# pmelchior/scarlet

Hardware: AMD Instinct MI355X
Metric: PGM iters/sec over batched blends; achieved HBM GB/s vs roofline (higher is better)
Workload: dtype f32; 1 GPU; configs[2]: 1024 independent 5-band 128x128 blends in total, 10 ExtendedSource components (41x41) each, ConvolutionRenderer FFT 160x160; iterations 0..1234 of a fit from the initial parameters; loop=blend, blends_total=1024, components_per_blend=10, sub_ranges_per_gpu=3

## Files before the change

scarlet_amd/csrc/fused_conv.hip:

```cpp
#include <cstdlib>
#include <type_traits>

#include "common.h"
#include "fft_regs.h"

namespace smi {

using fftk::cf;
using fftk::cmul;
using fftk::cmulc;
using fftk::ld;
using fftk::st;

namespace {

#ifndef SMI_CONV_THREADS
#define SMI_CONV_THREADS 1024
#endif
constexpr int kThreads = SMI_CONV_THREADS;
constexpr int kF2 = 16;

constexpr int conv_column_stride(int fy) { return ((fy + fy / kF2 + 3) / 8) * 8 + 4; }
constexpr size_t conv_lds_bytes(int fy, int fx) {
    return sizeof(float2) * ((size_t)(fx / 2) * conv_column_stride(fy) + 2 * fy + fx) +
           sizeof(double) * (kThreads / 64);
}

template <int FY1, int FX1, int ZB>
struct Cfg {
    static constexpr int FY = FY1 * kF2, FX = FX1 * kF2;
    static constexpr int NY1 = FY1 - ZB, NX1 = FX1 - ZB;
    static_assert(ZB >= 0 && NY1 >= 1 && NX1 >= 1, "padding blocks");
    static constexpr int NKX = FX / 2 + 1, NT = FX / 2;
    static constexpr int SY = conv_column_stride(FY);
    static_assert(SY >= FY + FY / kF2 && SY % 8 == 4, "column stride");
    static constexpr size_t lds_bytes = conv_lds_bytes(FY, FX);
};

__device__ __forceinline__ int sk(int y) { return y + (y >> 4); }

template <int F1, bool INV, int LIVE>
__device__ __forceinline__ void pass_stride_col(float2 *a, int n2, const cf (&tw)[F1]) {
    cf v[F1];
#pragma unroll
    for (int n1 = 0; n1 < F1; ++n1) {
        v[n1] = (INV || n1 < LIVE) ? ld(a[(kF2 + 1) * n1 + n2]) : cf{0.f, 0.f};
        if (INV && n1 > 0) v[n1] = cmulc(v[n1], tw[n1]);
    }
    fftk::Dft<F1, INV>::run(v);
#pragma unroll
    for (int k1 = 0; k1 < F1; ++k1) {
        if (INV && k1 >= LIVE) continue;
        if (!INV && k1 > 0) v[k1] = cmul(v[k1], tw[k1]);
        a[(kF2 + 1) * k1 + n2] = st(v[k1]);
    }
}

__device__ __forceinline__ void wave_lds_fence() {
    asm volatile("s_waitcnt lgkmcnt(0)" ::: "memory");
}

__host__ __device__ __forceinline__ int column_of(int kx, int Fx) {
    const int fx1 = Fx / kF2;
    return 2 * kx == Fx ? kx : 8 * (kx % fx1) + kx / fx1;
}

template <int F1>
__device__ __forceinline__ int pos(int k) {
    return kF2 * (k % F1) + k / F1;
}

__device__ __forceinline__ void wave_partial(double v, double *part) {
    for (int o = 32; o > 0; o >>= 1) v += __shfl_xor(v, o, 64);
    if ((threadIdx.x & 63) == 0) part[threadIdx.x >> 6] = v;
}
__device__ __forceinline__ double sum_partials(const double *part) {
    double t = 0.0;
    for (int i = 0; i < kThreads / 64; ++i) t += part[i];
    return t;
}

__device__ __forceinline__ void lds_barrier() {
    asm volatile("s_waitcnt lgkmcnt(0)\n\ts_barrier" ::: "memory");
}

using plane_t = __amdgpu_buffer_rsrc_t;
__device__ __forceinline__ plane_t band_plane(const float *p, int n_elements) {
    return __builtin_amdgcn_make_buffer_rsrc(const_cast<float *>(p), 0, n_elements * 4, 0x00020000);
}
__device__ __forceinline__ void plane_store(plane_t r, int y, int x, int W, float value) {
    const uint32_t off = x < W ? (uint32_t)(y * W + x) * 4u : 0x80000000u;
    __builtin_amdgcn_raw_buffer_store_b32(__builtin_bit_cast(uint32_t, value), r, off, 0, 0);
}
__device__ __forceinline__ float plane_load(plane_t r, int y, int x, int W) {
    const uint32_t off = x < W ? (uint32_t)(y * W + x) * 4u : 0x80000000u;
    return __builtin_bit_cast(float, __builtin_amdgcn_raw_buffer_load_b32(r, off, 0, 0));
}
struct PairRows {
    uint32_t o0, o1;
};
__device__ __forceinline__ PairRows pair_rows(int y, int n2, int W) {
    PairRows a;
    a.o0 = (uint32_t)(y * W + n2) * 4u;
    a.o1 = a.o0 + (uint32_t)W * 4u;
    asm volatile("" : "+v"(a.o0), "+v"(a.o1));
    return a;
}
template <int N1>
__device__ __forceinline__ void dw_load(const char *plane, uint32_t o, cf &d, cf &w) {
    const float4 t = *reinterpret_cast<const float4 *>(plane + (size_t)o + 16u * kF2 * N1);
    d = cf{t.x, t.y};
    w = cf{t.z, t.w};
}
template <int N1>
__device__ __forceinline__ cf pair_load(plane_t r, PairRows a) {
    return cf{__builtin_bit_cast(float, __builtin_amdgcn_raw_buffer_load_b32(r, a.o0 + 4u * kF2 * N1, 0, 0)),
              __builtin_bit_cast(float, __builtin_amdgcn_raw_buffer_load_b32(r, a.o1 + 4u * kF2 * N1, 0, 0))};
}

template <int FY1, int FX1, int ZB>
struct Conv {
    using C = Cfg<FY1, FX1, ZB>;
    static constexpr int NX1 = C::NX1;
    float2 *T, *twy, *twx, *qtab;
    int tid, n_pairs;

    __device__ __forceinline__ void zero_tail(float2 *a, int g) const {
        for (int y = 2 * n_pairs + g; y < kF2 * C::NY1; y += kF2) a[sk(y)] = make_float2(0.f, 0.f);
    }

    __device__ __forceinline__ void columns(const float2 *Kt, bool conj) {
        const int g = tid & (kF2 - 1), G = tid >> 4;
        const int col = 8 * (G >> 3) + ((G >> 1) & 3) + 4 * (G & 1);
        constexpr int kStep = kThreads / kF2;
        cf tw[FY1];
#pragma unroll
        for (int k1 = 0; k1 < FY1; ++k1) tw[k1] = ld(twy[kF2 * k1 + g]);
        for (int kt = col; kt < C::NT; kt += kStep) {
            const int kx = kt < 32 ? kt ^ 16 : kt;
            float2 *a = T + kx * C::SY;
            pass_stride_col<FY1, false, C::NY1>(a, g, tw);
            wave_lds_fence();
            if (g < FY1) {
                float2 *blk = a + (kF2 + 1) * g;
                const float2 *kp = Kt + (int64_t)kx * C::FY + kF2 * g;
                cf v[kF2], kv[kF2];
#pragma unroll
                for (int j = 0; j < kF2; ++j) kv[j] = ld(kp[j]);
#pragma unroll
                for (int j = 0; j < kF2; ++j) v[j] = ld(blk[j]);
                fftk::Dft<kF2, false>::run(v);
                if (kx == 0) {
#pragma unroll
                    for (int j = 0; j < kF2; ++j) blk[j] = st(v[j]);
                }
#pragma unroll
                for (int j = 0; j < kF2; ++j) v[j] = conj ? cmulc(v[j], kv[j]) : cmul(v[j], kv[j]);
                if (kx == 0) {
                    wave_lds_fence();
                    const float2 *base = g == 0 ? a + 1 : a + (kF2 + 1) * (FY1 - g);
                    const float2 *base0 = g == 0 ? a - 15 : base;
                    const float2 *qb = qtab + kF2 * g;
#pragma unroll
                    for (int j = 0; j < kF2; ++j) {
                        const cf m = ld((j == 0 ? base0 : base)[15 - j]), q = ld(qb[j]);
                        v[j] += conj ? cmul(cf{q.x, -q.y}, cf{m.x, -m.y}) : cmulc(q, m);
                        if (j % 4 == 3) __builtin_amdgcn_sched_barrier(0);
                    }
                    wave_lds_fence();
                }
                fftk::Dft<kF2, true>::run(v);
#pragma unroll
                for (int j = 0; j < kF2; ++j) blk[j] = st(v[j]);
            }
            wave_lds_fence();
            pass_stride_col<FY1, true, C::NY1>(a, g, tw);
            zero_tail(a, g);
        }
        lds_barrier();
    }

    struct StrideItem {
        int j, n2, zb;
        bool on;
    };
    __device__ __forceinline__ StrideItem stride_item(int it) const {
        StrideItem s;
        s.n2 = it & 15;
        s.j = it >> 4;
        s.on = s.j < n_pairs;
        s.zb = (s.n2 >> 1) * C::SY + sk(2 * s.j + (s.n2 & 1));
        return s;
    }
    __device__ __forceinline__ int stride_items() const { return n_pairs * kF2; }
    __device__ __forceinline__ void stride_twiddles(cf (&tw)[FX1], const StrideItem &s) const {
#pragma unroll
        for (int k1 = 1; k1 < FX1; ++k1) tw[k1] = ld(twx[kF2 * k1 + s.n2]);
    }
    __device__ __forceinline__ void stride_forward(cf *v, const StrideItem &s, const cf (&tw)[FX1]) {
        float2 *a = T + s.zb;
#pragma unroll
        for (int n1 = NX1; n1 < FX1; ++n1) v[n1] = cf{0.f, 0.f};
        fftk::Dft<FX1, false>::run(v);
#pragma unroll
        for (int k1 = 0; k1 < FX1; ++k1) {
            if (k1 > 0) v[k1] = cmul(v[k1], tw[k1]);
            a[8 * C::SY * k1] = st(v[k1]);
        }
    }
    __device__ __forceinline__ void stride_forward(cf *v, const StrideItem &s) {
        cf tw[FX1];
        stride_twiddles(tw, s);
        stride_forward(v, s, tw);
    }
    __device__ __forceinline__ void stride_inverse(cf *v, const StrideItem &s, const cf (&tw)[FX1]) {
        const float2 *a = T + s.zb;
#pragma unroll
        for (int n1 = 0; n1 < FX1; ++n1) {
            v[n1] = ld(a[8 * C::SY * n1]);
            if (n1 > 0) v[n1] = cmulc(v[n1], tw[n1]);
        }
        fftk::Dft<FX1, true>::run(v);
    }
    __device__ __forceinline__ void stride_inverse(cf *v, const StrideItem &s) {
        cf tw[FX1];
        stride_twiddles(tw, s);
        stride_inverse(v, s, tw);
    }

    static constexpr int kDouble = (FX1 - 1) / 2;
    static constexpr int kSlots = FX1 + (FX1 & 1);
    static constexpr int kGroupsPerTrip = (kThreads / 32) / kSlots;
    static_assert(kGroupsPerTrip >= 1, "slots of a pair group in one trip");
    static __device__ __forceinline__ int slot_block(int slot) {
        if (slot < 2 * kDouble) return (slot & 1) ? FX1 - (slot / 2 + 1) : slot / 2 + 1;
        return slot == 2 * kDouble ? 0 : FX1 / 2;
    }
    struct BlockItem {
        int z;
        int kind;
        bool wave_on;
    };
    BlockItem first;
    __device__ __forceinline__ BlockItem block_item(int group0) const {
        BlockItem b;
        const int grp = tid >> 5;
        const int slot = grp % kSlots;
        int j = (tid & 31) + 32 * (group0 + grp / kSlots);
        const int wgrp = __builtin_amdgcn_readfirstlane(tid >> 6) * 2;
        b.wave_on = wgrp < kGroupsPerTrip * kSlots && 32 * (group0 + wgrp / kSlots) < n_pairs;
        if (j >= n_pairs) j = n_pairs - 1;
        const int k1 = slot < FX1 ? slot_block(slot) : 0;
        b.z = 8 * k1 * C::SY + sk(2 * j);
        b.kind = slot < 2 * kDouble ? 0 : k1 == 0 ? 1 : 2;
        return b;
    }
    __device__ __forceinline__ void first_block_item() {
        first = block_item(0);
        asm volatile("" : "+v"(first.z), "+v"(first.kind));
    }
    __device__ __forceinline__ BlockItem trip_item(int trip) const {
        return trip == 0 ? first : block_item(trip * kGroupsPerTrip);
    }
    __device__ __forceinline__ int block_trips() const {
        if (kGroupsPerTrip >= (C::FY / 2 + 31) / 32) return 1;
        return ((n_pairs + 31) / 32 + kGroupsPerTrip - 1) / kGroupsPerTrip;
    }
    static __device__ __forceinline__ cf from_partner(cf v) {
        return cf{__shfl_xor(v.x, 32, 64), __shfl_xor(v.y, 32, 64)};
    }
    static __device__ __forceinline__ void sep(cf za, cf zb, cf &xa, cf &xb) {
        asm("v_pk_add_f32 %0, %1, %2 neg_hi:[0,1]" : "=v"(xa) : "v"(za), "v"(zb));
        asm("v_pk_add_f32 %0, %1, %2 op_sel:[1,1] op_sel_hi:[0,0] neg_hi:[1,0]" : "=v"(xb) : "v"(za), "v"(zb));
    }
    static __device__ __forceinline__ cf plus(cf xa, cf xb) {
        cf r;
        asm("v_pk_add_f32 %0, %1, %2 op_sel:[0,1] op_sel_hi:[1,0] neg_lo:[0,1]" : "=v"(r) : "v"(xa), "v"(xb));
        return r;
    }
    static __device__ __forceinline__ cf minus(cf xa, cf xb) {
        cf r;
        asm("v_pk_add_f32 %0, %1, %2 op_sel:[0,1] op_sel_hi:[1,0] neg_hi:[1,0]" : "=v"(r) : "v"(xa), "v"(xb));
        return r;
    }

    __device__ __forceinline__ void blocks_forward() {
        const int trips = block_trips();
        for (int trip = 0; trip < trips; ++trip) {
            const BlockItem b = trip_item(trip);
            if (!b.wave_on) continue;
            float2 *z = T + b.z;
            cf va[kF2], xa[8], xb[8];
#pragma unroll
            for (int i = 0; i < 8; ++i) {
                va[2 * i] = ld(z[i * C::SY]);
                va[2 * i + 1] = ld(z[i * C::SY + 1]);
            }
            fftk::Dft<kF2, false>::run(va);
            auto store = [&] {
#pragma unroll
                for (int k2 = 0; k2 < 8; ++k2) {
                    z[k2 * C::SY] = st(xa[k2]);
                    z[k2 * C::SY + 1] = st(xb[k2]);
                }
            };
            if (b.kind == 0) {
#pragma unroll
                for (int k2 = 0; k2 < 8; ++k2) sep(va[k2], from_partner(va[15 - k2]), xa[k2], xb[k2]);
                store();
            } else if (b.kind == 1) {
#pragma unroll
                for (int k2 = 0; k2 < 8; ++k2) sep(va[k2], va[(16 - k2) & 15], xa[k2], xb[k2]);
                cf na, nb;
                sep(va[8], va[8], na, nb);
                xa[0].y = na.x;
                xb[0].y = nb.x;
                store();
            } else {
#pragma unroll
                for (int k2 = 0; k2 < 8; ++k2) sep(va[k2], va[15 - k2], xa[k2], xb[k2]);
                store();
            }
        }
        lds_barrier();
    }

    template <typename F>
    __device__ __forceinline__ void blocks_inverse(F &&mid) {
        const int trips = block_trips();
        for (int trip = 0; trip < trips; ++trip) {
            const BlockItem b = trip_item(trip);
            if (!b.wave_on) {
                if (trip == 0) mid();
                continue;
            }
            float2 *z = T + b.z;
            cf va[kF2], xa[8], xb[8];
#pragma unroll
            for (int k2 = 0; k2 < 8; ++k2) {
                xa[k2] = ld(z[k2 * C::SY]);
                xb[k2] = ld(z[k2 * C::SY + 1]);
            }
            __builtin_amdgcn_sched_barrier(0);
            if (trip == 0) mid();
            __builtin_amdgcn_sched_barrier(0);
            auto tail = [&] {
                fftk::Dft<kF2, true>::run(va);
#pragma unroll
                for (int i = 0; i < 8; ++i) {
                    z[i * C::SY] = st(va[2 * i]);
                    z[i * C::SY + 1] = st(va[2 * i + 1]);
                }
            };
            if (b.kind == 0) {
#pragma unroll
                for (int k2 = 0; k2 < 8; ++k2) {
                    va[k2] = plus(xa[k2], xb[k2]);
                    va[15 - k2] = from_partner(minus(xa[k2], xb[k2]));
                }
                tail();
            } else if (b.kind == 1) {
                va[0] = cf{xa[0].x, xb[0].x};
                va[8] = cf{xa[0].y, xb[0].y};
#pragma unroll
                for (int k2 = 1; k2 < 8; ++k2) {
                    va[k2] = plus(xa[k2], xb[k2]);
                    va[16 - k2] = minus(xa[k2], xb[k2]);
                }
                tail();
            } else {
#pragma unroll
                for (int k2 = 0; k2 < 8; ++k2) {
                    va[k2] = plus(xa[k2], xb[k2]);
                    va[15 - k2] = minus(xa[k2], xb[k2]);
                }
                tail();
            }
        }
        lds_barrier();
    }
};


template <int FX1, int NX1, int M>
struct ModelGather {
    static constexpr uint32_t kNone = 0x40000000u;
    const BatchView &v;
    int band_c, H, W, y, n2, ylo;
    struct Lanes {
        int oy, ox, h, w, mo;
        float sd;
    };
    __device__ __forceinline__ int open(unsigned long long &todo, const Lanes &l, float &sd,
                                        cf (&mv)[M]) const {
        const bool none = todo == 0;
        const int kl = none ? 0 : __builtin_ctzll(todo);
        todo &= todo - 1;
        const int oy = __builtin_amdgcn_readlane(l.oy, kl), hh = __builtin_amdgcn_readlane(l.h, kl);
        const int ox = __builtin_amdgcn_readlane(l.ox, kl), w = __builtin_amdgcn_readlane(l.w, kl);
        const float *mbase = v.morph + __builtin_amdgcn_readlane(l.mo, kl);
        const plane_t r = band_plane(mbase, hh * w);
        sd = __builtin_bit_cast(float, __builtin_amdgcn_readlane(__builtin_bit_cast(int, l.sd), kl));
        const int n1lo = (ox > 0 ? ox : 0) >> 4;
        const uint32_t hlim = none ? 0u : (uint32_t)min(hh, H - oy);
        const uint32_t wlim4 = 4u * (uint32_t)min(w, W - ox);
        const uint32_t ry = (uint32_t)(y - oy), w4 = 4u * (uint32_t)w;
        uint32_t row0, row1;
        asm("v_mul_u32_u24 %0, %1, %2" : "=v"(row0) : "v"(ry), "s"(w4));
        asm("v_mul_u32_u24 %0, %1, %2" : "=v"(row1) : "v"(ry + 1u), "s"(w4));
        row0 = ry < hlim ? row0 : kNone;
        row1 = ry + 1u < hlim ? row1 : kNone;
        const uint32_t x4 = (uint32_t)(16 * n1lo + n2 - ox) * 4u;
#pragma unroll
        for (int m = 0; m < M; ++m) {
            uint32_t t = x4 + 64u * m;
            t = t < wlim4 ? t : kNone;
            mv[m].x = __builtin_bit_cast(float, __builtin_amdgcn_raw_buffer_load_b32(r, row0 + t, 0, 0));
            mv[m].y = __builtin_bit_cast(float, __builtin_amdgcn_raw_buffer_load_b32(r, row1 + t, 0, 0));
        }
        return none ? -1 : n1lo;
    }
    __device__ __forceinline__ void close(int n1lo_, float sd_, const cf (&mv)[M], cf (&acc)[FX1]) const {
        const cf sd = cf{sd_, sd_};
        fftk::static_for<0, NX1>([&](auto lo) {
            constexpr int n1lo = decltype(lo)::value;
            if (n1lo_ == n1lo) {
#pragma unroll
                for (int m = 0; m < M; ++m)
                    if (n1lo + m < NX1) acc[n1lo + m] = fftk::fma2(mv[m], sd, acc[n1lo + m]);
                asm volatile("; n1lo = %0" ::"n"(n1lo));
            }
        });
    }
    __device__ __forceinline__ void run(int b, int lane, cf (&acc)[FX1]) const {
#pragma unroll
        for (int n1 = 0; n1 < NX1; ++n1) acc[n1] = cf{0.f, 0.f};
        const int cs = v.comp_start[b], ce = v.comp_start[b + 1];
        for (int kb = cs; kb < ce; kb += 64) {
            const int kk = kb + lane;
            const bool have = kk < ce;
            Lanes l;
            l.oy = have ? v.c_oy[kk] : 0;
            l.ox = have ? v.c_ox[kk] : 0;
            l.h = have ? v.c_h[kk] : 0;
            l.w = have ? v.c_w[kk] : 0;
            l.mo = have ? (int)v.c_moff[kk] : 0;
            l.sd = have ? v.sed[kk * v.C + band_c] : 0.f;
            const bool hit = have && l.oy < ylo + 8 && l.oy + l.h > ylo && l.oy < H && l.ox < W &&
                             l.ox + l.w > 0;
            unsigned long long todo = __ballot(hit);
            if (!todo) continue;
            cf mva[M], mvb[M];
            float sda, sdb;
            int na = open(todo, l, sda, mva);
            for (;;) {
                const int nb = open(todo, l, sdb, mvb);
                close(na, sda, mva, acc);
                if (nb < 0) break;
                na = open(todo, l, sda, mva);
                close(nb, sdb, mvb, acc);
                if (na < 0) break;
            }
        }
    }
};

extern __shared__ __attribute__((aligned(16))) float2 lds_conv[];

template <int FY1, int FX1, int ZB, bool EXT>
__global__ __launch_bounds__(kThreads) void fused_conv_kernel(BatchView v, const float *model,
                                                              const float2 *Kt, int k_bands,
                                                              int k_per_blend, float *out,
                                                              int mode, long long *dbg) {
    using C = Cfg<FY1, FX1, ZB>;
    constexpr int NX1 = C::NX1;
    const int total = gridDim.x;
    int lid = blockIdx.x;
    if (total % 8 == 0) lid = (blockIdx.x % 8) * (total / 8) + blockIdx.x / 8;
    const int b = lid / v.C + v.blend0, c = lid % v.C;
    if (v.state[b] >= 2) return;
    const int tid = threadIdx.x;
    const int H = v.H, W = v.W;
    const int Hb = EXT ? v.frame_h(b) : H, Wb = EXT ? v.frame_w(b) : W;

    Conv<FY1, FX1, ZB> cv;
    cv.T = lds_conv;
    cv.twy = cv.T + C::NT * C::SY;
    cv.twx = cv.twy + C::FY;
    cv.tid = tid;
    cv.n_pairs = (H + 1) / 2;
    cv.first_block_item();
    cv.qtab = cv.twx + C::FX;
    double *loss_part = reinterpret_cast<double *>(cv.qtab + C::FY);
    const int64_t band = ((int64_t)b * v.C + c) * H * W;
    const int n_items = cv.stride_items();
    using Item = typename Conv<FY1, FX1, ZB>::StrideItem;

    const bool have_cube = model != nullptr;
    const plane_t r_model = band_plane(have_cube ? model + band : v.data + band, H * W);
    cf mrow[FX1];
    auto fetch_model = [&](const Item &s) {
        const PairRows a = pair_rows(2 * s.j, s.n2, W);
        fftk::static_for<0, NX1>([&](auto n1c) {
            constexpr int n1 = decltype(n1c)::value;
            mrow[n1] = pair_load<n1>(r_model, a);
        });
    };
    auto render_rows = [&](const Item &s) {
        const int j0 = __builtin_amdgcn_readfirstlane(s.j - ((tid & 63) >> 4));
        if (v.render_slots <= 4) {
            const ModelGather<FX1, NX1, 4> g{v, c, Hb, Wb, 2 * s.j, s.n2, 2 * j0};
            g.run(b, tid & 63, mrow);
        } else {
            const ModelGather<FX1, NX1, (FX1 < 6 ? FX1 : 6)> g{v, c, Hb, Wb, 2 * s.j, s.n2, 2 * j0};
            g.run(b, tid & 63, mrow);
        }
    };
    if (have_cube) fetch_model(cv.stride_item(tid));
    for (int j = tid; j < C::FY; j += kThreads) {
        float s, co;
        sincospif(2.0f * (float)((j / kF2) * (j % kF2)) / (float)C::FY, &s, &co);
        cv.twy[j] = make_float2(co, -s);
    }
    for (int j = tid; j < C::FX; j += kThreads) {
        float s, co;
        sincospif(2.0f * (float)((j / kF2) * (j % kF2)) / (float)C::FX, &s, &co);
        cv.twx[j] = make_float2(co, -s);
    }
    {
        const int y0 = 2 * cv.n_pairs, tail = kF2 * C::NY1 - y0;
        for (int i = tid; i < tail * C::NT; i += kThreads)
            cv.T[(i / tail) * C::SY + sk(y0 + i % tail)] = make_float2(0.f, 0.f);
    }
    const float2 *K = Kt + ((int64_t)(k_per_blend ? b : 0) * k_bands + (k_bands == 1 ? 0 : c)) *
                               C::FY * C::NKX;
    for (int j = tid; j < C::FY; j += kThreads) cv.qtab[j] = K[(int64_t)(C::FX / 2) * C::FY + j];
    __syncthreads();
#ifndef SMI_DBG_BLOCK
#define SMI_DBG_BLOCK 0
#endif
#define SMI_STAMP(i) if (dbg && tid == 0 && blockIdx.x == SMI_DBG_BLOCK) dbg[i] = clock64()
    SMI_STAMP(0);

    for (int it = tid; (have_cube ? it : it - (tid & 63)) < n_items; it += kThreads) {
        const Item s = cv.stride_item(it);
        if (have_cube) {
            if (it != tid) fetch_model(s);
#pragma unroll
            for (int n1 = 0; n1 < NX1; ++n1)
                if (kF2 * n1 + s.n2 >= W) mrow[n1] = cf{0.f, 0.f};
        } else {
            render_rows(s);
        }
        if (s.on) cv.stride_forward(mrow, s);
    }
    lds_barrier();
    SMI_STAMP(6);
    cv.blocks_forward();
    SMI_STAMP(1);
    cv.columns(K, false);
    SMI_STAMP(2);
    double loss = 0.0;
    {
        cf loss2 = cf{0.f, 0.f};
        const int64_t pband = ((int64_t)b * v.C + c) * cv.n_pairs * W;
        const char *p_dw = reinterpret_cast<const char *>(v.dw + pband);
        const plane_t r_rendered = band_plane(out + band, H * W);
#ifndef SMI_CONV_PRE
#define SMI_CONV_PRE 8
#endif
        constexpr int kPre = SMI_CONV_PRE < NX1 ? SMI_CONV_PRE : NX1;
        cf dv[NX1], wv[NX1];
        auto fetch = [&](const Item &s, auto from, auto to) {
            uint32_t o = (uint32_t)(min(s.j, cv.n_pairs - 1) * W + s.n2) * 16u;
            asm volatile("" : "+v"(o));
            fftk::static_for<decltype(from)::value, decltype(to)::value>([&](auto n1c) {
                constexpr int n1 = decltype(n1c)::value;
                dw_load<n1>(p_dw, o, dv[n1], wv[n1]);
            });
        };
        using std::integral_constant;
        const Item s0 = cv.stride_item(tid);
        fetch(s0, integral_constant<int, 0>{}, integral_constant<int, kPre>{});
        constexpr int kLate = NX1 > 8 ? NX1 - 8 : 0;
        cv.blocks_inverse([&] { fetch(s0, integral_constant<int, kPre>{}, integral_constant<int, NX1 - kLate>{}); });
        SMI_STAMP(10);
        for (int it = tid; it < n_items; it += kThreads) {
            const Item s = cv.stride_item(it);
            const int y = 2 * s.j;
            if (it != tid) fetch(s, integral_constant<int, 0>{}, integral_constant<int, NX1 - kLate>{});
            cf m[FX1];
            cv.stride_inverse(m, s);
            fetch(s, integral_constant<int, NX1 - kLate>{}, integral_constant<int, NX1>{});
#pragma unroll
            for (int n1 = 0; n1 < NX1; ++n1) {
                const int x = kF2 * n1 + s.n2;
                if (mode == 1) {
                    plane_store(r_rendered, y, x, W, m[n1].x);
                    plane_store(r_rendered, y + 1, x, W, m[n1].y);
                }
                const cf w = x < W ? wv[n1] : cf{0.f, 0.f};
                const cf d = m[n1] - dv[n1];
                m[n1] = w * d;
                loss2 = fftk::fma2(m[n1], d, loss2);
            }
            cv.stride_forward(m, s);
            loss += (double)loss2.x + (double)loss2.y;
            loss2 = cf{0.f, 0.f};
        }
        wave_partial(loss, loss_part);
        lds_barrier();
        SMI_STAMP(11);
        cv.blocks_forward();
    }
    if (tid == 0) v.loss_partial[(int64_t)b * v.n_partial + c] = sum_partials(loss_part);
    SMI_STAMP(3);
    if (mode == 1) return;
    cv.columns(K, true);
    SMI_STAMP(4);
    {
        const plane_t r_out = band_plane(out + band, H * W);
        cv.blocks_inverse([] {});
        SMI_STAMP(12);
        for (int it = tid; it < n_items; it += kThreads) {
            const Item s = cv.stride_item(it);
            cf g[FX1];
            cv.stride_inverse(g, s);
#pragma unroll
            for (int k1 = 0; k1 < NX1; ++k1) {
                plane_store(r_out, 2 * s.j, kF2 * k1 + s.n2, W, g[k1].x);
                plane_store(r_out, 2 * s.j + 1, kF2 * k1 + s.n2, W, g[k1].y);
            }
        }
    }
    SMI_STAMP(5);
#undef SMI_STAMP
}

#ifndef SMI_CONV_SHORT_ROWS
template <int FY1>
__global__ void permute_kernel_spectrum(const float2 *Khat, float2 *Kt, int NKX, float scale) {
    const int Fx = 2 * (NKX - 1);
    constexpr int FY = FY1 * kF2;
    const int img = blockIdx.y;
    const int i = blockIdx.x * blockDim.x + threadIdx.x;
    if (i >= FY * NKX) return;
    const int ky = i / NKX, kx = i - ky * NKX;
    const float2 k = Khat[(int64_t)img * FY * NKX + i];
    Kt[((int64_t)img * NKX + column_of(kx, Fx)) * FY + pos<FY1>(ky)] =
        make_float2(k.x * scale, k.y * scale);
}

__global__ void pack_dc_nyquist(float2 *Kt, int Fy, int NKX) {
    const int i = blockIdx.x * blockDim.x + threadIdx.x;
    if (i >= Fy) return;
    float2 *k0 = Kt + (int64_t)blockIdx.y * NKX * Fy + i, *kn = k0 + (int64_t)(NKX - 1) * Fy;
    const float2 a = *k0, b = *kn;
    *k0 = make_float2(0.5f * (a.x + b.x), 0.5f * (a.y + b.y));
    *kn = make_float2(0.5f * (a.x - b.x), 0.5f * (a.y - b.y));
}

__global__ void stamp_dft_x(const float *kern, double2 *A, int ph, int pw, int Fx, int NKX) {
    const int img = blockIdx.y;
    const int i = blockIdx.x * blockDim.x + threadIdx.x;
    if (i >= ph * NKX) return;
    const int dy = i / NKX, kx = i - dy * NKX;
    double re = 0.0, im = 0.0;
    for (int dx = 0; dx < pw; ++dx) {
        int t = (kx * (dx - pw / 2)) % Fx;
        if (t < 0) t += Fx;
        double s, c;
        sincospi(2.0 * (double)t / (double)Fx, &s, &c);
        const double k = (double)kern[((int64_t)img * ph + dy) * pw + dx];
        re += k * c;
        im -= k * s;
    }
    A[(int64_t)img * ph * NKX + i] = make_double2(re, im);
}

template <int FY1>
__global__ void stamp_dft_y(const double2 *A, float2 *Kt, int ph, int NKX, double scale) {
    constexpr int FY = FY1 * kF2;
    const int img = blockIdx.y;
    const int i = blockIdx.x * blockDim.x + threadIdx.x;
    if (i >= FY * NKX) return;
    const int ky = i / NKX, kx = i - ky * NKX;
    double re = 0.0, im = 0.0;
    for (int dy = 0; dy < ph; ++dy) {
        int t = (ky * (dy - ph / 2)) % FY;
        if (t < 0) t += FY;
        double s, c;
        sincospi(2.0 * (double)t / (double)FY, &s, &c);
        const double2 a = A[((int64_t)img * ph + dy) * NKX + kx];
        re += a.x * c + a.y * s;
        im += a.y * c - a.x * s;
    }
    Kt[((int64_t)img * NKX + column_of(kx, 2 * (NKX - 1))) * FY + pos<FY1>(ky)] =
        make_float2((float)(re * scale), (float)(im * scale));
}

#endif

template <int FY1, int FX1, int ZB, bool EXT>
int launch_ext(const BatchView &v, const float *model, const float2 *Kt, int k_bands,
               int k_per_blend, float *out, int mode, long long *dbg, hipStream_t s) {
    using C = Cfg<FY1, FX1, ZB>;
    auto kern = fused_conv_kernel<FY1, FX1, ZB, EXT>;
    static size_t configured[kMaxDevices] = {};
    if (int rc = ensure_dynamic_lds(reinterpret_cast<const void *>(kern), C::lds_bytes, configured))
        return rc;
    hipLaunchKernelGGL(kern, dim3(v.nb * v.C), dim3(kThreads), C::lds_bytes, s, v, model, Kt,
                       k_bands, k_per_blend, out, mode, dbg);
    return SMI_OK;
}

template <int FY1, int FX1, int ZB>
int launch_zb(const BatchView &v, const float *model, const float2 *Kt, int k_bands,
              int k_per_blend, float *out, int mode, long long *dbg, hipStream_t s) {
    if (v.frame_hw)
        return launch_ext<FY1, FX1, ZB, true>(v, model, Kt, k_bands, k_per_blend, out, mode, dbg, s);
    return launch_ext<FY1, FX1, ZB, false>(v, model, Kt, k_bands, k_per_blend, out, mode, dbg, s);
}

template <int FY1, int FX1>
int launch_impl(const BatchView &v, const float *model, const float2 *Kt, int k_bands,
                int k_per_blend, float *out, int mode, long long *dbg, hipStream_t s) {
    const int zy = FY1 - (v.H + kF2 - 1) / kF2, zx = FX1 - (v.W + kF2 - 1) / kF2;
    const int zb = zy < zx ? zy : zx;
    if (zb >= 2) return launch_zb<FY1, FX1, 2>(v, model, Kt, k_bands, k_per_blend, out, mode, dbg, s);
    if (zb == 1) return launch_zb<FY1, FX1, 1>(v, model, Kt, k_bands, k_per_blend, out, mode, dbg, s);
    return launch_zb<FY1, FX1, 0>(v, model, Kt, k_bands, k_per_blend, out, mode, dbg, s);
}

}

#ifndef SMI_CONV_SHORT_ROWS
bool fused_conv_supported(int Fy, int Fx) {
    auto ok = [](int f) { return f == 64 || f == 80 || f == 96 || f == 128 || f == 160; };
    if (!ok(Fy) || !ok(Fx)) return false;
    return conv_lds_bytes(Fy, Fx) <= 160 * 1024;
}

int fused_conv_length(int n) {
    for (int f : {64, 80, 96, 128, 160})
        if (f >= n) return f;
    return 0;
}

#endif

#define SMI_FUSED_DISPATCH(FN, ...)                                             \
    switch (Fy / 16 * 100 + Fx / 16) {                                          \
        case 404: return FN<4, 4>(__VA_ARGS__);                  \
        case 405: return FN<4, 5>(__VA_ARGS__);                  \
        case 406: return FN<4, 6>(__VA_ARGS__);                  \
        case 408: return FN<4, 8>(__VA_ARGS__);                  \
        case 410: return FN<4, 10>(__VA_ARGS__);                 \
        case 504: return FN<5, 4>(__VA_ARGS__);                  \
        case 505: return FN<5, 5>(__VA_ARGS__);                  \
        case 506: return FN<5, 6>(__VA_ARGS__);                  \
        case 508: return FN<5, 8>(__VA_ARGS__);                  \
        case 510: return FN<5, 10>(__VA_ARGS__);                 \
        case 604: return FN<6, 4>(__VA_ARGS__);                  \
        case 605: return FN<6, 5>(__VA_ARGS__);                  \
        case 606: return FN<6, 6>(__VA_ARGS__);                  \
        case 608: return FN<6, 8>(__VA_ARGS__);                  \
        case 610: return FN<6, 10>(__VA_ARGS__);                 \
        case 804: return FN<8, 4>(__VA_ARGS__);                  \
        case 805: return FN<8, 5>(__VA_ARGS__);                  \
        case 806: return FN<8, 6>(__VA_ARGS__);                  \
        case 808: return FN<8, 8>(__VA_ARGS__);                  \
        case 810: return FN<8, 10>(__VA_ARGS__);                 \
        case 1004: return FN<10, 4>(__VA_ARGS__);                \
        case 1005: return FN<10, 5>(__VA_ARGS__);                \
        case 1006: return FN<10, 6>(__VA_ARGS__);                \
        case 1008: return FN<10, 8>(__VA_ARGS__);                \
        case 1010: return FN<10, 10>(__VA_ARGS__);               \
        default: break;                                                         \
    }

#ifdef SMI_CONV_SHORT_ROWS
int launch_fused_conv_short(const BatchView &v, int Fy, int Fx, const float *model,
                            const float2 *Kt, int k_bands, int k_per_blend, float *out, int mode,
                            long long *dbg, hipStream_t s) {
    SMI_FUSED_DISPATCH(launch_impl, v, model, Kt, k_bands, k_per_blend, out, mode, dbg, s)
    set_error("fused convolution: FFT shape not instantiated");
    return SMI_ERR_INVALID;
}
#else
bool fused_conv_instantiated(int Fy, int Fx) { return fused_conv_supported(Fy, Fx); }

bool fused_conv_choose(int ny, int nx, int *Fy, int *Fx) {
    long best = 0;
    for (int fy : {64, 80, 96, 128, 160})
        for (int fx : {64, 80, 96, 128, 160}) {
            if (fy < ny || fx < nx || !fused_conv_supported(fy, fx)) continue;
            if (!best || (long)fy * fx < best) {
                best = (long)fy * fx;
                *Fy = fy;
                *Fx = fx;
            }
        }
    return best != 0;
}

int launch_fused_conv(const BatchView &v, int Fy, int Fx, const float *model, const float2 *Kt,
                      int k_bands, int k_per_blend, float *out, int mode, long long *dbg,
                      hipStream_t s) {
    static const char *force = getenv("SMI_CONV_WORKGROUP");
    const bool large = (Fx == 160 && Fy >= 80) || (Fy == 160 && Fx >= 128);
    if (force ? force[0] == '5' : !large)
        return launch_fused_conv_short(v, Fy, Fx, model, Kt, k_bands, k_per_blend, out, mode, dbg, s);
    SMI_FUSED_DISPATCH(launch_impl, v, model, Kt, k_bands, k_per_blend, out, mode, dbg, s)
    set_error("fused convolution: FFT shape not instantiated");
    return SMI_ERR_INVALID;
}

int launch_stamp_spectrum(const float *d_kern, double2 *d_tmp, float2 *Kt, int n_img, int ph,
                          int pw, int Fy, int Fx, double scale, hipStream_t s) {
    const int NKX = Fx / 2 + 1;
    hipLaunchKernelGGL(stamp_dft_x, dim3((ph * NKX + 255) / 256, n_img), dim3(256), 0, s, d_kern,
                       d_tmp, ph, pw, Fx, NKX);
    const dim3 grid((Fy * NKX + 255) / 256, n_img);
    switch (Fy / 16) {
        case 4: hipLaunchKernelGGL(stamp_dft_y<4>, grid, dim3(256), 0, s, d_tmp, Kt, ph, NKX, scale); break;
        case 5: hipLaunchKernelGGL(stamp_dft_y<5>, grid, dim3(256), 0, s, d_tmp, Kt, ph, NKX, scale); break;
        case 6: hipLaunchKernelGGL(stamp_dft_y<6>, grid, dim3(256), 0, s, d_tmp, Kt, ph, NKX, scale); break;
        case 8: hipLaunchKernelGGL(stamp_dft_y<8>, grid, dim3(256), 0, s, d_tmp, Kt, ph, NKX, scale); break;
        case 10: hipLaunchKernelGGL(stamp_dft_y<10>, grid, dim3(256), 0, s, d_tmp, Kt, ph, NKX, scale); break;
        default:
            set_error("stamp spectrum: unsupported FFT height");
            return SMI_ERR_INVALID;
    }
    hipLaunchKernelGGL(pack_dc_nyquist, dim3((Fy + 255) / 256, n_img), dim3(256), 0, s, Kt, Fy, NKX);
    return SMI_OK;
}

int launch_permute_kernel_spectrum(const float2 *Khat, float2 *Kt, int n_img, int Fy, int Fx,
                                   float scale, hipStream_t s) {
    const int NKX = Fx / 2 + 1;
    const dim3 grid((Fy * NKX + 255) / 256, n_img);
    switch (Fy / 16) {
        case 4: hipLaunchKernelGGL(permute_kernel_spectrum<4>, grid, dim3(256), 0, s, Khat, Kt, NKX, scale); break;
        case 5: hipLaunchKernelGGL(permute_kernel_spectrum<5>, grid, dim3(256), 0, s, Khat, Kt, NKX, scale); break;
        case 6: hipLaunchKernelGGL(permute_kernel_spectrum<6>, grid, dim3(256), 0, s, Khat, Kt, NKX, scale); break;
        case 8: hipLaunchKernelGGL(permute_kernel_spectrum<8>, grid, dim3(256), 0, s, Khat, Kt, NKX, scale); break;
        case 10: hipLaunchKernelGGL(permute_kernel_spectrum<10>, grid, dim3(256), 0, s, Khat, Kt, NKX, scale); break;
        default:
            set_error("permute_kernel_spectrum: unsupported FFT height");
            return SMI_ERR_INVALID;
    }
    hipLaunchKernelGGL(pack_dc_nyquist, dim3((Fy + 255) / 256, n_img), dim3(256), 0, s, Kt, Fy, NKX);
    return SMI_OK;
}

#endif

}
```

Measured before the change: 1.504 million blend-iterations/s.

## Prefetch first render gather before twiddle setup and use static full-row slots

Result: slower. 1.446 million blend-iterations/s (-3.9%).

```diff
diff --git a/scarlet_amd/csrc/fused_conv.hip b/scarlet_amd/csrc/fused_conv.hip
--- a/scarlet_amd/csrc/fused_conv.hip
+++ b/scarlet_amd/csrc/fused_conv.hip
@@ -382,17 +382,32 @@
 };
 
 
-template <int FX1, int NX1, int M>
+constexpr bool render_static_slots(int fy1, int fx1, int zb) {
+    return !(fx1 == 5 || (fy1 == 5 && fx1 == 6));
+}
+
+struct RenderLanes {
+    int oy, ox, h, w, mo;
+    float sd;
+};
+struct RenderHead {
+    int cs, ce;
+    unsigned long long todo;
+    RenderLanes l;
+};
+template <int FX1, int NX1, int M, bool STATIC>
 struct ModelGather {
     static constexpr uint32_t kNone = 0x40000000u;
+    static constexpr int S = STATIC ? NX1 : M;
     const BatchView &v;
     int band_c, H, W, y, n2, ylo;
-    struct Lanes {
-        int oy, ox, h, w, mo;
+    using Lanes = RenderLanes;
+    struct Slots {
+        cf mv[S];
         float sd;
+        int n1lo;
     };
-    __device__ __forceinline__ int open(unsigned long long &todo, const Lanes &l, float &sd,
-                                        cf (&mv)[M]) const {
+    __device__ __forceinline__ void open(unsigned long long &todo, const Lanes &l, Slots &o) const {
         const bool none = todo == 0;
         const int kl = none ? 0 : __builtin_ctzll(todo);
         todo &= todo - 1;
@@ -400,8 +415,8 @@
         const int ox = __builtin_amdgcn_readlane(l.ox, kl), w = __builtin_amdgcn_readlane(l.w, kl);
         const float *mbase = v.morph + __builtin_amdgcn_readlane(l.mo, kl);
         const plane_t r = band_plane(mbase, hh * w);
-        sd = __builtin_bit_cast(float, __builtin_amdgcn_readlane(__builtin_bit_cast(int, l.sd), kl));
-        const int n1lo = (ox > 0 ? ox : 0) >> 4;
+        o.sd = __builtin_bit_cast(float, __builtin_amdgcn_readlane(__builtin_bit_cast(int, l.sd), kl));
+        const int n1lo = STATIC ? 0 : (ox > 0 ? ox : 0) >> 4;
         const uint32_t hlim = none ? 0u : (uint32_t)min(hh, H - oy);
         const uint32_t wlim4 = 4u * (uint32_t)min(w, W - ox);
         const uint32_t ry = (uint32_t)(y - oy), w4 = 4u * (uint32_t)w;
@@ -412,56 +427,82 @@
         row1 = ry + 1u < hlim ? row1 : kNone;
         const uint32_t x4 = (uint32_t)(16 * n1lo + n2 - ox) * 4u;
 #pragma unroll
-        for (int m = 0; m < M; ++m) {
+        for (int m = 0; m < S; ++m) {
             uint32_t t = x4 + 64u * m;
             t = t < wlim4 ? t : kNone;
-            mv[m].x = __builtin_bit_cast(float, __builtin_amdgcn_raw_buffer_load_b32(r, row0 + t, 0, 0));
-            mv[m].y = __builtin_bit_cast(float, __builtin_amdgcn_raw_buffer_load_b32(r, row1 + t, 0, 0));
-        }
-        return none ? -1 : n1lo;
-    }
-    __device__ __forceinline__ void close(int n1lo_, float sd_, const cf (&mv)[M], cf (&acc)[FX1]) const {
-        const cf sd = cf{sd_, sd_};
-        fftk::static_for<0, NX1>([&](auto lo) {
-            constexpr int n1lo = decltype(lo)::value;
-            if (n1lo_ == n1lo) {
-#pragma unroll
-                for (int m = 0; m < M; ++m)
-                    if (n1lo + m < NX1) acc[n1lo + m] = fftk::fma2(mv[m], sd, acc[n1lo + m]);
-                asm volatile("; n1lo = %0" ::"n"(n1lo));
-            }
-        });
+            o.mv[m].x = __builtin_bit_cast(float, __builtin_amdgcn_raw_buffer_load_b32(r, row0 + t, 0, 0));
+            o.mv[m].y = __builtin_bit_cast(float, __builtin_amdgcn_raw_buffer_load_b32(r, row1 + t, 0, 0));
+        }
+        o.n1lo = none ? -1 : n1lo;
+    }
+    __device__ __forceinline__ void close(const Slots &o, cf (&acc)[FX1]) const {
+        const cf sd = cf{o.sd, o.sd};
+        if constexpr (STATIC) {
+#pragma unroll
+            for (int n1 = 0; n1 < NX1; ++n1) acc[n1] = fftk::fma2(o.mv[n1], sd, acc[n1]);
+        } else {
+            fftk::static_for<0, NX1>([&](auto lo) {
+                constexpr int n1lo = decltype(lo)::value;
+                if (o.n1lo == n1lo) {
+#pragma unroll
+                    for (int m = 0; m < M; ++m)
+                        if (n1lo + m < NX1) acc[n1lo + m] = fftk::fma2(o.mv[m], sd, acc[n1lo + m]);
+                    asm volatile("; n1lo = %0" ::"n"(n1lo));
+                }
+            });
+        }
+    }
+    __device__ __forceinline__ unsigned long long group(int kb, int ce, int lane, Lanes &l) const {
+        const int kk = kb + lane;
+        const bool have = kk < ce;
+        l.oy = have ? v.c_oy[kk] : 0;
+        l.ox = have ? v.c_ox[kk] : 0;
+        l.h = have ? v.c_h[kk] : 0;
+        l.w = have ? v.c_w[kk] : 0;
+        l.mo = have ? (int)v.c_moff[kk] : 0;
+        l.sd = have ? v.sed[kk * v.C + band_c] : 0.f;
+        const bool hit = have && l.oy < ylo + 8 && l.oy + l.h > ylo && l.oy < H && l.ox < W &&
+                         l.ox + l.w > 0;
+        return __ballot(hit);
+    }
+    __device__ __forceinline__ void walk(unsigned long long &todo, const Lanes &l, Slots &a,
+                                         cf (&acc)[FX1]) const {
+        Slots b;
+        for (;;) {
+            open(todo, l, b);
+            close(a, acc);
+            if (b.n1lo < 0) break;
+            open(todo, l, a);
+            close(b, acc);
+            if (a.n1lo < 0) break;
+        }
+    }
+    __device__ __forceinline__ void begin(int b, int lane, RenderHead &h, Slots &a) const {
+        h.cs = v.comp_start[b];
+        h.ce = v.comp_start[b + 1];
+        h.todo = group(h.cs, h.ce, lane, h.l);
+        open(h.todo, h.l, a);
+    }
+    __device__ __forceinline__ void finish(int lane, RenderHead &h, Slots &a, cf (&acc)[FX1]) const {
+#pragma unroll
+        for (int n1 = 0; n1 < NX1; ++n1) acc[n1] = cf{0.f, 0.f};
+        if (a.n1lo >= 0) walk(h.todo, h.l, a, acc);
+        rest(h.cs + 64, h.ce, lane, acc);
+    }
+    __device__ __forceinline__ void rest(int kb0, int ce, int lane, cf (&acc)[FX1]) const {
+        for (int kb = kb0; kb < ce; kb += 64) {
+            Lanes l;
+            unsigned long long todo = group(kb, ce, lane, l);
+            if (!todo) continue;
+            Slots a;
+            open(todo, l, a);
+            walk(todo, l, a, acc);
+        }
     }
     __device__ __forceinline__ void run(int b, int lane, cf (&acc)[FX1]) const {
 #pragma unroll
         for (int n1 = 0; n1 < NX1; ++n1) acc[n1] = cf{0.f, 0.f};
-        const int cs = v.comp_start[b], ce = v.comp_start[b + 1];
-        for (int kb = cs; kb < ce; kb += 64) {
-            const int kk = kb + lane;
-            const bool have = kk < ce;
-            Lanes l;
-            l.oy = have ? v.c_oy[kk] : 0;
-            l.ox = have ? v.c_ox[kk] : 0;
-            l.h = have ? v.c_h[kk] : 0;
-            l.w = have ? v.c_w[kk] : 0;
-            l.mo = have ? (int)v.c_moff[kk] : 0;
-            l.sd = have ? v.sed[kk * v.C + band_c] : 0.f;
-            const bool hit = have && l.oy < ylo + 8 && l.oy + l.h > ylo && l.oy < H && l.ox < W &&
-                             l.ox + l.w > 0;
-            unsigned long long todo = __ballot(hit);
-            if (!todo) continue;
-            cf mva[M], mvb[M];
-            float sda, sdb;
-            int na = open(todo, l, sda, mva);
-            for (;;) {
-                const int nb = open(todo, l, sdb, mvb);
-                close(na, sda, mva, acc);
-                if (nb < 0) break;
-                na = open(todo, l, sda, mva);
-                close(nb, sdb, mvb, acc);
-                if (na < 0) break;
-            }
-        }
+        rest(v.comp_start[b], v.comp_start[b + 1], lane, acc);
     }
 };
 
@@ -506,17 +547,42 @@
             mrow[n1] = pair_load<n1>(r_model, a);
         });
     };
-    auto render_rows = [&](const Item &s) {
+#ifndef SMI_DBG_BLOCK
+#define SMI_DBG_BLOCK 0
+#endif
+#define SMI_STAMP(i) if (dbg && tid == 0 && blockIdx.x == SMI_DBG_BLOCK) dbg[i] = clock64()
+    SMI_STAMP(7);
+    constexpr bool kStatic = render_static_slots(FY1, FX1, ZB);
+    constexpr bool kHead = kStatic;
+    using Gather4 = ModelGather<FX1, NX1, 4, kStatic>;
+    using Gather6 = ModelGather<FX1, NX1, (FX1 < 6 ? FX1 : 6), kStatic>;
+    RenderHead head;
+    typename Gather4::Slots head_slots;
+    auto render_rows = [&](const Item &s, bool first) {
         const int j0 = __builtin_amdgcn_readfirstlane(s.j - ((tid & 63) >> 4));
-        if (v.render_slots <= 4) {
-            const ModelGather<FX1, NX1, 4> g{v, c, Hb, Wb, 2 * s.j, s.n2, 2 * j0};
-            g.run(b, tid & 63, mrow);
+        auto render = [&](auto g, auto &slots) {
+            if (kHead && first)
+                g.finish(tid & 63, head, slots, mrow);
+            else
+                g.run(b, tid & 63, mrow);
+        };
+        if constexpr (kStatic) {
+            render(Gather4{v, c, Hb, Wb, 2 * s.j, s.n2, 2 * j0}, head_slots);
+        } else if (v.render_slots <= 4) {
+            render(Gather4{v, c, Hb, Wb, 2 * s.j, s.n2, 2 * j0}, head_slots);
         } else {
-            const ModelGather<FX1, NX1, (FX1 < 6 ? FX1 : 6)> g{v, c, Hb, Wb, 2 * s.j, s.n2, 2 * j0};
-            g.run(b, tid & 63, mrow);
+            typename Gather6::Slots slots;
+            render(Gather6{v, c, Hb, Wb, 2 * s.j, s.n2, 2 * j0}, slots);
         }
     };
-    if (have_cube) fetch_model(cv.stride_item(tid));
+    if (have_cube) {
+        fetch_model(cv.stride_item(tid));
+    } else if (kHead) {
+        const Item s = cv.stride_item(tid);
+        const int j0 = __builtin_amdgcn_readfirstlane(s.j - ((tid & 63) >> 4));
+        const Gather4 g{v, c, Hb, Wb, 2 * s.j, s.n2, 2 * j0};
+        g.begin(b, tid & 63, head, head_slots);
+    }
     for (int j = tid; j < C::FY; j += kThreads) {
         float s, co;
         sincospif(2.0f * (float)((j / kF2) * (j % kF2)) / (float)C::FY, &s, &co);
@@ -536,10 +602,6 @@
                                C::FY * C::NKX;
     for (int j = tid; j < C::FY; j += kThreads) cv.qtab[j] = K[(int64_t)(C::FX / 2) * C::FY + j];
     __syncthreads();
-#ifndef SMI_DBG_BLOCK
-#define SMI_DBG_BLOCK 0
-#endif
-#define SMI_STAMP(i) if (dbg && tid == 0 && blockIdx.x == SMI_DBG_BLOCK) dbg[i] = clock64()
     SMI_STAMP(0);
 
     for (int it = tid; (have_cube ? it : it - (tid & 63)) < n_items; it += kThreads) {
@@ -550,7 +612,8 @@
             for (int n1 = 0; n1 < NX1; ++n1)
                 if (kF2 * n1 + s.n2 >= W) mrow[n1] = cf{0.f, 0.f};
         } else {
-            render_rows(s);
+            render_rows(s, it == tid);
+            if (it == tid) SMI_STAMP(8);
         }
         if (s.on) cv.stride_forward(mrow, s);
     }
```
